# Bissmella/Small-object-detection-transformers

Measured on AMD Instinct MI355X. Metric: images/sec (1024x1024 RGB+IR) train fwd+bwd, higher is better.
Workload: dtype bf16; 1 GPU; SRyolo_MF.yaml (model.yaml graph), batch 8/GPU @ 1024x1024 RGB+IR, fwd + hand-written bwd + fused SGD-nesterov/weight-decay + EMA step, loss = YOLOv5 ComputeLoss (CIoU + BCE, device kernels), 32 synthetic boxes/image, random-init weights; global_batch=8, parallelism=dp1

## Files before the change

### include/sodt_hip.h

```cpp
#ifndef SODT_HIP_H
#define SODT_HIP_H
#include <stddef.h>
#include <stdint.h>

#ifdef __cplusplus
extern "C" {
#endif

typedef struct ihipStream_t* sodt_stream_t;

#define SODT_F32 0
#define SODT_BF16 1
#define SODT_MAX_SEG 9

typedef struct {
  const void* p;
  int ld;
  int klen;
  int dy, dx;
  int mul, shr;
  int Hi, Wi;
} sodt_seg;

typedef struct {
// ... 18 lines not shown
#define SODT_EPI_DRELU 4096

typedef struct {
  sodt_aspec a;
  const void* W; int ldw;
  void* C; int ldc;
  void* C2; int ldc2;
  const float* bias;
  const void* R; int ldr; int rmod;
  const void* aux; int ldaux;
  double* stats;
  const float* scale; const float* shift;
  int M, N, K, flags;
  int oscatter, omul, ody, odx, OH, OW;
  int det_na, det_no, det_hw;
} sodt_gemm_args;

int sodt_gemm_nt(const sodt_gemm_args* g, int dtype, sodt_stream_t st);
int sodt_gemm_set_variant(int force_tiled);

typedef struct {
  const void* dY; int ldy;
  sodt_aspec x;
  float* dW; int lddw;
  float* dbias;
  int M, N, K;
  int kperm_c, kperm_t;
  int splits;
  float* partial;
  long partial_floats;
} sodt_gemm_tn_args;

int sodt_gemm_tn(const sodt_gemm_tn_args* g, int dtype, sodt_stream_t st);

int sodt_layernorm_fwd(const void* x, const float* gamma, const float* beta, void* y, float* stats,
                       int M, int C, int dtype, sodt_stream_t st);
int sodt_layernorm_bwd(const void* dy, const void* x, const float* stats, const float* gamma,
                       const void* dres, void* dx, float* dgamma, float* dbeta,
                       int M, int C, int dtype, sodt_stream_t st);

int sodt_window_attn_fwd(const void* qkv, const float* bias_t, void* out, float* lse,
                         int B, int H, int W, int C, int heads, int ws, int shift,
                         int dtype, sodt_stream_t st);
int sodt_window_attn_bwd(const void* qkv, const float* bias_t, const void* out, const void* dout,
                         const float* lse, void* dqkv, float* dbias_t, float* dq_acc,
                         int B, int H, int W, int C, int heads, int ws, int shift,
                         int dtype, sodt_stream_t st);

int sodt_bilinear_up2_fwd(const void* x, void* y, int ldy, int B, int H, int W, int C, int dtype, sodt_stream_t st);
int sodt_bilinear_up2_bwd(const void* dy, int lddy, void* dx, const void* relu_out, int B, int H, int W, int C, int dtype,
                          sodt_stream_t st);
int sodt_pixel_shuffle2(const void* in, void* out, int B, int H, int W, int C, int inverse, int dtype, sodt_stream_t st);
int sodt_add_rows(void* dst, int ldd, int dcol, const void* src, int lds, int scol, long M, int C, int dtype, sodt_stream_t st);
int sodt_nchw_f32_from_rows(const void* rows, int ld, float* y, int B, int C, int H, int W, int dtype, sodt_stream_t st);
int sodt_rows_from_nchw_f32(const float* y, void* rows, int ld, int B, int C, int H, int W, int dtype, sodt_stream_t st);

int sodt_conv3x3_c64n8_fwd(const void* x, const void* w, const float* bias, void* y, float* y_nchw, int B, int H, int W, int cout, int dtype,
                           sodt_stream_t st);
int sodt_conv3x3_c64n8_dgrad(const void* dy, const float* dy_nchw, const void* wT, void* dx, int B, int H, int W, int cout, int dtype,
                             sodt_stream_t st);
int sodt_conv3x3_c64n8_wgrad(const void* dy, const float* dy_nchw, const void* x, float* dw, float* db, float* scratch, int B, int H, int W,
                             int cout, int dtype, sodt_stream_t st);
long sodt_conv3x3_c64n8_wgrad_scratch_bytes(void);

typedef struct {
  int w_row_stride, w_row_off;
// ... 195 lines not shown
```

### small-object-detection-transformers_amd/_lib.py

```python
from __future__ import annotations

import ctypes as C
import os

HERE = os.path.dirname(os.path.abspath(__file__))
DEFAULT_LIB_PATH = os.path.join(HERE, "libsodt_hip.so")
LIB_PATH = os.environ.get("SODT_LIB_PATH") or DEFAULT_LIB_PATH
DIAGNOSTIC_ENV = ("SODT_LIB_PATH", "SODT_HG_DBG", "SODT_WMSA_ONE_WAVE")


def overrides():
    return {k: os.environ[k] for k in DIAGNOSTIC_ENV if os.environ.get(k)}

MAX_SEG = 9
F32, BF16 = 0, 1
U8 = 2
SR_MODES = {"IR": 0, "RGB": 1, "RGB+IR": 2}
EPI_BIAS, EPI_RESID, EPI_GELU_DUAL, EPI_DGELU = 1, 2, 4, 8
EPI_STATS, EPI_AFFINE_SILU, EPI_DETECT, EPI_OUT_F32 = 16, 32, 64, 128
EPI_GELU, EPI_DGELU_RC, EPI_RELU, EPI_DRELU = 256, 512, 2048, 4096
STATS_REPL = 16


class Seg(C.Structure):
    _fields_ = [("p", C.c_void_p), ("ld", C.c_int), ("klen", C.c_int), ("dy", C.c_int), ("dx", C.c_int),
                ("mul", C.c_int), ("shr", C.c_int), ("Hi", C.c_int), ("Wi", C.c_int)]


class ASpec(C.Structure):
    _fields_ = [("s", Seg * MAX_SEG), ("nseg", C.c_int), ("spatial", C.c_int), ("Ho", C.c_int), ("Wo", C.c_int)]


class GemmArgs(C.Structure):
    _fields_ = [("a", ASpec),
                ("W", C.c_void_p), ("ldw", C.c_int),
                ("C", C.c_void_p), ("ldc", C.c_int),
                ("C2", C.c_void_p), ("ldc2", C.c_int),
                ("bias", C.c_void_p),
                ("R", C.c_void_p), ("ldr", C.c_int), ("rmod", C.c_int),
                ("aux", C.c_void_p), ("ldaux", C.c_int),
                ("stats", C.c_void_p),
                ("scale", C.c_void_p), ("shift", C.c_void_p),
                ("M", C.c_int), ("N", C.c_int), ("K", C.c_int), ("flags", C.c_int),
                ("oscatter", C.c_int), ("omul", C.c_int), ("ody", C.c_int), ("odx", C.c_int),
                ("OH", C.c_int), ("OW", C.c_int),
                ("det_na", C.c_int), ("det_no", C.c_int), ("det_hw", C.c_int)]


class GemmTnArgs(C.Structure):
    _fields_ = [("dY", C.c_void_p), ("ldy", C.c_int),
                ("x", ASpec),
                ("dW", C.c_void_p), ("lddw", C.c_int),
                ("dbias", C.c_void_p),
                ("M", C.c_int), ("N", C.c_int), ("K", C.c_int),
                ("kperm_c", C.c_int), ("kperm_t", C.c_int), ("splits", C.c_int),
                ("partial", C.c_void_p), ("partial_floats", C.c_long)]


class StepCtl(C.Structure):
    _fields_ = [("acc_sumsq", C.c_double), ("acc_found", C.c_uint), ("ticket", C.c_uint),
                ("sumsq", C.c_double), ("grad_norm", C.c_double), ("step", C.c_longlong),
                ("found_inf", C.c_float), ("inv_scale_eff", C.c_float), ("clip_coef", C.c_float), ("skip", C.c_int),
                ("reserved", C.c_int * 2)]


class PrepDesc(C.Structure):
    _fields_ = [("src", C.c_void_p), ("dst", C.c_void_p),
                ("d0", C.c_int), ("d1", C.c_int), ("d2", C.c_int),
                ("p0", C.c_int), ("p1", C.c_int), ("p2", C.c_int),
                ("dst_ld", C.c_int), ("inner_ld", C.c_int)]


_P, _I, _L, _F = C.c_void_p, C.c_int, C.c_long, C.c_float
class Conv3Geo(C.Structure):
    _fields_ = [("w_row_stride", C.c_int), ("w_row_off", C.c_int), ("in_mul", C.c_int), ("in_i", C.c_int), ("in_j", C.c_int),
                ("out_mul", C.c_int), ("out_i", C.c_int), ("out_j", C.c_int)]


SIGNATURES = {
    "sodt_nms_candidates": [_P, _I, _I, C.c_float, _I, _P, _P, _I, _P, _P],
    "sodt_nms_workspace_bytes": [_L, C.POINTER(C.c_size_t)],
    "sodt_nms_select": [_P, _I, _P, _L, C.c_float, _I, _P, C.c_size_t, _P, _P, _P, _P],
    "sodt_wbf_candidates": [_P, _I, _I, _I, _F, _F, _P, _P, _P, _P, _P, _P],
    "sodt_wbf_fuse_workspace_bytes": [_I, _L, C.POINTER(C.c_size_t)],
    "sodt_wbf_fuse": [_P, _P, _P, _P, _P, _P, _I, _L, C.POINTER(C.c_double), _I, C.c_double, _F, _I, _I, _I, _P, C.c_size_t,
                      _P, _P, _P, _P, _P, _P],
    "sodt_eval_match_workspace_bytes": [_I, _L, _L, C.POINTER(C.c_size_t)],
    "sodt_eval_match": [_P, _P, _I, _L, _P, _L, _P, C.POINTER(C.c_float), _P, C.c_size_t, _P, _P, _P],
    "sodt_ap_per_class_workspace_bytes": [_L, _L, _I, C.POINTER(C.c_size_t)],
    "sodt_ap_per_class": [_P, _P, _P, _L, _P, _L, _I, _P, C.c_size_t, _P, _P, _P, _P, _P, _P, _P, _P],
    "sodt_confusion_update_workspace_bytes": [_I, _L, _L, C.POINTER(C.c_size_t)],
    "sodt_confusion_update": [_P, _P, _I, _L, _P, _L, _P, _I, _F, _F, _P, C.c_size_t, _P, _P, _P],
    "sodt_gemm_nt": [C.POINTER(GemmArgs), _I, _P],
    "sodt_gemm_tn": [C.POINTER(GemmTnArgs), _I, _P],
    "sodt_layernorm_fwd": [_P, _P, _P, _P, _P, _I, _I, _I, _P],
    "sodt_layernorm_bwd": [_P, _P, _P, _P, _P, _P, _P, _P, _I, _I, _I, _P],
    "sodt_window_attn_fwd": [_P, _P, _P, _P, _I, _I, _I, _I, _I, _I, _I, _I, _P],
    "sodt_window_attn_bwd": [_P, _P, _P, _P, _P, _P, _P, _P, _I, _I, _I, _I, _I, _I, _I, _I, _P],
    "sodt_wmsa_pack": [_P, _P, _P, _P, _P, _P, _P, _P, _P, _P, _I, _I, _I, _I, _P],
    "sodt_wmsa_block_fwd": [_P, _P, _P, _P, _P, _P, _P, _P, _P, _P, _I, _I, _I, _I, _I, _I, _I, _I, _P],
    "sodt_window_attn_bwd_wm": [_P, _P, _P, _P, _P, _P, _I, _I, _I, _I, _I, _I, _I, _I, _P],
    "sodt_wmsa_block_bwd": [_P, _P, _P, _P, _P, _P, _P, _I, _I, _I, _I, _I, _I, _I, _I, _P],
    "sodt_frontend_fwd": [_P, _P, _L, _P, _P, _P, _P, _P, _I, _I, _I, _I, _P],
    "sodt_frontend_bwd": [_P, _P, _L, _P, _P, _P, _P, _P, _P, _P, _P, _P, _I, _I, _I, _P, _L, _I, _P],
    "sodt_patch_embed4_fwd": [_P, _P, _L, _P, _P, _P, _I, _I, _P],
    "sodt_patch_embed4_bwd": [_P, _P, _L, _P, _P, _P, _I, _I, _P],
    "sodt_cross_attn_ln_fwd": [_P, _P, _P, _P, _I, _I, _I, _I, _I, _P],
    "sodt_cross_attn_ln_bwd": [_P, _P, _P, _P, _P, _P, _I, _I, _I, _I, _I, _P],
    "sodt_bn_finalize": [_P, _P, _P, _P, _L, _I, _F, _F, _P],
    "sodt_bn_affine": [_P, _P, _P, _P, _P, _I, _P],
    "sodt_bn_silu_fwd": [_P, _P, _P, _P, _P, _I, _L, _I, _I, _P],
    "sodt_bn_silu_bwd_reduce": [_P, _I, _P, _P, _P, _P, _P, _L, _I, _I, _P],
    "sodt_bn_silu_bwd_apply": [_P, _I, _P, _P, _P, _P, _P, _P, _P, _P, _L, _I, _I, _P],
    "sodt_copy_rows": [_P, _I, _P, _I, _I, _I, _I, _I, _I, _I, _P],
    "sodt_gather_sum_rows": [_P, _I, _P, _I, _I, _I, _I, _I, _I, _I, _I, _P],
    "sodt_detect_unpermute": [_P, _P, _I, _I, _I, _I, _I, _I, _P],
    "sodt_detect_decode": [_P, _P, _P, _I, _I, _I, _I, _I, _F, _P],
    "sodt_prep_weights": [_P, _I, _I, _I, _P],
    "sodt_transpose_f32": [_P, _P, _I, _I, _I, _P],
    "sodt_cast": [_P, _P, _L, _I, _I, _P],
    "sodt_batch_sum": [_P, _P, _I, _L, _I, _P],
    "sodt_memset_zero": [_P, _L, _P],
    "sodt_gemm_set_variant": [_I],
    "sodt_maxpool5_fwd": [_P, _I, _P, _I, _P, _I, _I, _I, _I, _I, _P],
    "sodt_maxpool5_bwd": [_P, _I, _P, _P, _I, _I, _I, _I, _I, _I, _I, _P],
    "sodt_yolo_loss_workspace_bytes": [_L, _I, _I, C.POINTER(C.c_size_t)],
    "sodt_yolo_loss": [_P, _P, _I, _P, _I, _I, _I, _I, _I, _F, _F, _F, _F, _F, _F, _F, _P, C.c_size_t, _P, _P, _P],
# ... 75 lines not shown
```

### small-object-detection-transformers_amd/engine.py

```python
from __future__ import annotations

import os

import ctypes as C
from typing import Dict, List, Optional, Tuple

import warnings

import torch

from . import _lib as L
from . import ops
from .ops import SegSpec

HEADS = 12
E = "image_encoder."
TAPS2 = ((0, 0), (0, 1), (1, 0), (1, 1))
TAPS3 = tuple((dy, dx) for dy in (-1, 0, 1) for dx in (-1, 0, 1))
MERGE = ((0, 0), (1, 0), (0, 1), (1, 1))
USE_HIPGRAPH = os.environ.get("SODT_HIPGRAPH", "0") == "1"


class Plan:
    def __init__(self, B, S, dt, training, dev):
# ... 99 lines not shown
        return None, None, None, None, None


class Engine:
    def __init__(self, model):
        self.model = model
        self.params: Dict[str, torch.nn.Parameter] = dict(model.named_parameters())
        self.buffers: Dict[str, torch.Tensor] = dict(model.named_buffers())
        p0 = next(iter(self.params.values()))
        if not p0.is_cuda:
            raise RuntimeError("move the model to the GPU first: the engine has no CPU path")
        for n, p in self.params.items():
            if p.dtype != torch.float32:
                raise RuntimeError(f"master parameters must be float32 (got {p.dtype} for {n}); call model.float()")
        self.dev = p0.device
        enc = model.image_encoder
        self.img_t = enc.pos_embed.shape[1]
        det = model.detect[-1]
        self.na, self.no, self.nc = det.na, det.no, det.nc
        self.det_np = (det.na * det.no + 15) // 16 * 16
        self.fused = not any(type(m).__name__ == "BatchNorm2d" for m in model.detect.modules())
        self.sr = bool(getattr(model, "sr", False))
        self._check_head()
        self.plans: Dict[Tuple, Plan] = {}
        self.probes_fwd: Optional[dict] = None
        self.probes_bwd: Optional[dict] = None
        self.prep: Dict[torch.dtype, dict] = {}
        self._build_grad_buffer()
        self._build_param_buffer()
        self._anchor = torch.zeros(1, device=self.dev, requires_grad=True)
        self.ddp = None
        self.use_fused_wmsa = True
        self.use_fused_mlp = True
        self.convmlp_fold_maxc = 384
        self.use_direct_conv3 = True
        self._tn_scratch = torch.empty(16 << 20, dtype=torch.float32, device=self.dev)
        ops.set_tn_scratch(self._tn_scratch)

    def _check_head(self):
        from . import model as M
        d = self.model.detect
        enc_c = (256, 256, 512)
        vals = {j: ([(("enc", j), enc_c[j], 0)], j) for j in range(3)}
        units, rules = [], {}
        uses: Dict[tuple, int] = {}

        def resolve(f, yi):
            j = yi - 1 if f == -1 else f
            if not isinstance(j, int) or j not in vals or j >= yi:
                raise NotImplementedError(f"head row {yi - 3}: input {f!r} does not name an earlier feature-list entry")
            return j
        if not isinstance(d[-1], M.Detect) or d[-1].nl != 1:
            raise NotImplementedError("the head must end in a one-layer Detect (models/model.yaml:74)")
        for k, m in enumerate(d):
            yi, kind = 3 + k, type(m).__name__
            if kind in ("Conv", "C3", "SPP"):
                if not isinstance(m.f, int):
                    raise NotImplementedError(f"head row {k}: {kind} takes one input")
                parts, level = vals[resolve(m.f, yi)]
                c1 = sum(c for _, c, _ in parts)
                if kind == "Conv":
                    kk, c2 = m.conv.kernel_size[0], m.conv.out_channels
                    if m.conv.in_channels != c1:
                        raise NotImplementedError(f"head row {k}: Conv expects {m.conv.in_channels} channels, graph gives {c1}")
                    if kk == 3 and len(parts) * 9 > L.MAX_SEG:
                        raise NotImplementedError(f"head row {k}: a 3x3 Conv on a concatenation needs {len(parts) * 9} K-segments (max {L.MAX_SEG})")
# ... 493 lines not shown
        elif pre in P["cmlp"]:
            cm = P["cmlp"][pre]
            ops.convmlp_compose(p[pre + "mlp.fc1.weight"], p[pre + "mlp.fc1.bias"], p[pre + "mlp.conv1.weight"], p[pre + "mlp.conv1.bias"],
                                cm["weff"], cm["weffT"], cm["beff"], cm["vtap"], Cc)
            cp = plan.buf(tag + ".cp", (M, Cc))
            ca = plan.buf(tag + ".ca", (M, Cc))
            segs = [SegSpec(xn2, Cc, 0, dy, dx, 1, 0, H, W) for (dy, dx) in TAPS2]
            ops.gemm_nt(segs, cm["weff"], cp, M, Cc, 4 * Cc, spatial=(H, W), bias=cm["beff"], gelu_out=ca)
            ops.convmlp_border_fix(cp, ca, cm["vtap"], B, H, W, Cc)
            ops.gemm_nt([SegSpec(ca)], w[pre + "mlp.fc2.weight"], xo, M, Cc, Cc, bias=p[pre + "mlp.fc2.bias"], resid=xm)
        else:
            u = plan.buf(tag + ".u", (M, Cc))
            ops.gemm_nt([SegSpec(xn2)], w[pre + "mlp.fc1.weight"], u, M, Cc, Cc, bias=p[pre + "mlp.fc1.bias"])
            cp = plan.buf(tag + ".cp", (M, Cc))
            ca = plan.buf(tag + ".ca", (M, Cc))
            segs = [SegSpec(u, Cc, 0, dy, dx, 1, 0, H, W) for (dy, dx) in TAPS2]
            ops.gemm_nt(segs, w[pre + "mlp.conv1.weight"], cp, M, Cc, 4 * Cc, spatial=(H, W), bias=p[pre + "mlp.conv1.bias"],
                        gelu_out=ca)
            ops.gemm_nt([SegSpec(ca)], w[pre + "mlp.fc2.weight"], xo, M, Cc, Cc, bias=p[pre + "mlp.fc2.bias"], resid=xm)
        plan.saved[tag] = dict(x_in=x_in, geo=(B, H, W, Cc, ws, shift), fused=fused, wpk=wpk, pad=(Hp, Wp) if padded else None)
        return xo

    def _block_bwd(self, plan, P, tag, blk, dY, dX):
        ops.set_tag(tag + ".bwd")
        p, wT, g, b = self.params, P["wT"], self.g, plan.bufs
        pre = E + tag + "."
        sv = plan.saved[tag]
        B, H, W, Cc, ws, shift = sv["geo"]
        M = B * H * W
        x_in = sv["x_in"]
        xm, xn2, xn1, ao = b[tag + ".xm"], b[tag + ".xn2"], b[tag + ".xn1"], b[tag + ".ao"]
        dxn = plan.buf(f"g.dxn.{Cc}", (M, Cc))
        dxm = plan.buf(f"g.dxm.{Cc}", (M, Cc))
        if blk.mlp.linear:
            ha = b[tag + ".ha"]
            dh = plan.buf(f"g.dh.{Cc}", (M, 4 * Cc))
            ops.gemm_tn(dY, [SegSpec(ha)], g[pre + "mlp.fc2.weight"], M, Cc, 4 * Cc, dbias=g[pre + "mlp.fc2.bias"])
            if (tag + ".hp") in b:
                ops.gemm_nt([SegSpec(dY)], wT[pre + "mlp.fc2.weight"], dh, M, 4 * Cc, Cc, dgelu_aux=b[tag + ".hp"])
            else:
                ops.gemm_nt([SegSpec(xn2), SegSpec(dY)], P["wcat"][pre + "mlp.fc1.weight"], dh, M, 4 * Cc, 2 * Cc,
                            bias=p[pre + "mlp.fc1.bias"], dgelu_rc=True)
            ops.gemm_tn(dh, [SegSpec(xn2)], g[pre + "mlp.fc1.weight"], M, 4 * Cc, Cc, dbias=g[pre + "mlp.fc1.bias"])
            dln2 = (dh, 4 * Cc)
        elif pre in P["cmlp"]:
            cm = P["cmlp"][pre]
            cp, ca = b[tag + ".cp"], b[tag + ".ca"]
            dc = plan.buf(f"g.dc.{Cc}", (M, Cc))
            ops.gemm_tn(dY, [SegSpec(ca)], g[pre + "mlp.fc2.weight"], M, Cc, Cc, dbias=g[pre + "mlp.fc2.bias"])
            ops.gemm_nt([SegSpec(dY)], wT[pre + "mlp.fc2.weight"], dc, M, Cc, Cc, dgelu_aux=cp)
            scr = plan.buf(f"g.cmlp.{Cc}", (Cc * 4 * Cc + 4 * Cc,), torch.float32)
            dweff, colsum, bs = scr[: Cc * 4 * Cc].view(Cc, 4 * Cc), scr[Cc * 4 * Cc: Cc * 4 * Cc + Cc], scr[Cc * 4 * Cc + Cc:].view(3, Cc)
            ops.zero_(scr)
            segs = [SegSpec(xn2, Cc, 0, dy, dx, 1, 0, H, W) for (dy, dx) in TAPS2]
            ops.gemm_tn(dc, segs, dweff, M, Cc, 4 * Cc, spatial=(H, W), dbias=colsum)
            ops.convmlp_border_sums(dc, bs, B, H, W, Cc)
            ops.convmlp_decompose(dweff, colsum, bs, p[pre + "mlp.fc1.weight"], p[pre + "mlp.fc1.bias"], p[pre + "mlp.conv1.weight"],
                                  g[pre + "mlp.conv1.weight"], g[pre + "mlp.conv1.bias"], g[pre + "mlp.fc1.weight"], g[pre + "mlp.fc1.bias"], Cc)
            dln2 = None
        else:
            u, cp, ca = b[tag + ".u"], b[tag + ".cp"], b[tag + ".ca"]
            dc = plan.buf(f"g.dc.{Cc}", (M, Cc))
            du = plan.buf(f"g.du.{Cc}", (M, Cc))
            ops.gemm_tn(dY, [SegSpec(ca)], g[pre + "mlp.fc2.weight"], M, Cc, Cc, dbias=g[pre + "mlp.fc2.bias"])
            ops.gemm_nt([SegSpec(dY)], wT[pre + "mlp.fc2.weight"], dc, M, Cc, Cc, dgelu_aux=cp)
            segs = [SegSpec(u, Cc, 0, dy, dx, 1, 0, H, W) for (dy, dx) in TAPS2]
            ops.gemm_tn(dc, segs, g[pre + "mlp.conv1.weight"], M, Cc, 4 * Cc, spatial=(H, W), dbias=g[pre + "mlp.conv1.bias"],
                        kperm=(Cc, 4))
            segs = [SegSpec(dc, Cc, 0, -dy, -dx, 1, 0, H, W) for (dy, dx) in TAPS2]
            ops.gemm_nt(segs, wT[pre + "mlp.conv1.weight"], du, M, Cc, 4 * Cc, spatial=(H, W))
            ops.gemm_tn(du, [SegSpec(xn2)], g[pre + "mlp.fc1.weight"], M, Cc, Cc, dbias=g[pre + "mlp.fc1.bias"])
            dln2 = (du, Cc)
        if dln2 is None:
            segs = [SegSpec(dc, Cc, 0, -dy, -dx, 1, 0, H, W) for (dy, dx) in TAPS2]
            ops.gemm_nt(segs, cm["weffT"], dxn, M, Cc, 4 * Cc, spatial=(H, W))
            ops.layernorm_bwd(dxn, xm, b[tag + ".st2"], p[pre + "norm2.weight"], dY, dxm, g[pre + "norm2.weight"], g[pre + "norm2.bias"], M, Cc)
        else:
            ops.gemm_nt([SegSpec(dln2[0])], wT[pre + "mlp.fc1.weight"], dxn, M, Cc, dln2[1])
            ops.layernorm_bwd(dxn, xm, b[tag + ".st2"], p[pre + "norm2.weight"], dY, dxm, g[pre + "norm2.weight"], g[pre + "norm2.bias"], M, Cc)
        if sv.get("pad"):
            self._padded_attn_bwd(plan, P, tag, pre, sv, dxm, dxn, dX)
            return
        ops.gemm_tn(dxm, [SegSpec(ao)], g[pre + "attn.proj.weight"], M, Cc, Cc, dbias=g[pre + "attn.proj.bias"])
        dao = dxn
        ops.gemm_nt([SegSpec(dxm)], wT[pre + "attn.proj.weight"], dao, M, Cc, Cc)
        dqkv = plan.buf(f"g.dqkv.{Cc}", (M, 3 * Cc))
        L2 = 2 * ws - 1
        dbt = plan.buf(f"g.dbt.{L2}", (HEADS, L2 * L2), torch.float32, zero=True)
        if sv["fused"] and plan.dt == torch.bfloat16:
            ops.wmsa_block_bwd(xn1, sv["wpk"], P["bias_t"][pre + "attn.relative_position_bias_table"], dao, b[tag + ".lsew"],
                               dqkv, dbt, B, H, W, Cc, HEADS, ws, shift)
        elif sv["fused"]:
            ops.window_attn_bwd_wm(b[tag + ".qkvw"], P["bias_t"][pre + "attn.relative_position_bias_table"], dao, b[tag + ".lsew"],
                                   dqkv, dbt, B, H, W, Cc, HEADS, ws, shift)
        else:
            scratch = plan.buf(f"g.attn_scratch.{Cc}", (M * (Cc + HEADS),), torch.float32, zero=True) if ws * ws > 64 else None
            ops.window_attn_bwd(b[tag + ".qkv"], P["bias_t"][pre + "attn.relative_position_bias_table"], ao, dao, b[tag + ".lse"], dqkv,
                                dbt, scratch, B, H, W, Cc, HEADS, ws, shift)
        ops.transpose_f32(dbt, g[pre + "attn.relative_position_bias_table"], HEADS, L2 * L2, accumulate=2)
        ops.gemm_tn(dqkv, [SegSpec(xn1)], g[pre + "attn.qkv.weight"], M, 3 * Cc, Cc, dbias=g[pre + "attn.qkv.bias"])
        ops.gemm_nt([SegSpec(dqkv)], wT[pre + "attn.qkv.weight"], dxn, M, Cc, 3 * Cc)
        ops.layernorm_bwd(dxn, x_in, b[tag + ".st1"], p[pre + "norm1.weight"], dxm, dX, g[pre + "norm1.weight"], g[pre + "norm1.bias"], M, Cc)

    def _padded_attn_bwd(self, plan, P, tag, pre, sv, dxm, dxn, dX):
        p, wT, g, b = self.params, P["wT"], self.g, plan.bufs
        B, H, W, Cc, ws, _ = sv["geo"]
        Hp, Wp = sv["pad"]
        M, Mp = B * H * W, B * Hp * Wp
        aop, qkv, lse = b[tag + ".aop"], b[tag + ".qkv"], b[tag + ".lse"]
        ops.gemm_tn(dxm, [SegSpec(aop, Cc, 0, 0, 0, 1, 0, Hp, Wp)], g[pre + "attn.proj.weight"], M, Cc, Cc, spatial=(H, W),
                    dbias=g[pre + "attn.proj.bias"])
        daop = plan.buf(f"g.daop.{Cc}", (Mp, Cc))
        ops.gemm_nt([SegSpec(dxm, Cc, 0, 0, 0, 1, 0, H, W)], wT[pre + "attn.proj.weight"], daop, Mp, Cc, Cc, spatial=(Hp, Wp))
        dqkv = plan.buf(f"g.dqkvp.{Cc}", (Mp, 3 * Cc))
        L2 = 2 * ws - 1
        dbt = plan.buf(f"g.dbt.{L2}", (HEADS, L2 * L2), torch.float32, zero=True)
        scratch = plan.buf(f"g.attn_scratchp.{Cc}", (Mp * (Cc + HEADS),), torch.float32, zero=True) if ws * ws > 64 else None
        ops.window_attn_bwd(qkv, P["bias_t"][pre + "attn.relative_position_bias_table"], aop, daop, lse, dqkv, dbt, scratch,
# ... 371 lines not shown
```

### small-object-detection-transformers_amd/ops.py

```python
from __future__ import annotations

import ctypes as C
from typing import List, Optional, Sequence, Tuple

import torch

from . import _lib as L

_lib = L.load()

_active_recorder: Optional[list] = None


class Recorder:

    def __init__(self):
        self.calls: List[Tuple] = []
        self.keep: List = []

    def __enter__(self):
        global _active_recorder
        assert _active_recorder is None, "nested recorders are not supported"
        _active_recorder = self.calls
        return self
# ... 199 lines not shown
    return max(1, min(M // 256 if M >= 256 else 1, max(1, slots // tiles)))


_tn_scratch: Optional[torch.Tensor] = None


def set_tn_scratch(t: Optional[torch.Tensor]) -> None:
    global _tn_scratch
    assert t is None or (t.dtype == torch.float32 and t.is_contiguous())
    _tn_scratch = t


def gemm_tn(dY: torch.Tensor, segs: Sequence[SegSpec], dW: torch.Tensor, M: int, N: int, K: int, *,
            ldy: Optional[int] = None, y_off: int = 0, spatial: Optional[Tuple[int, int]] = None,
            dbias: Optional[torch.Tensor] = None, lddw: Optional[int] = None, kperm: Optional[Tuple[int, int]] = None,
            splits: Optional[int] = None) -> None:
    g = L.GemmTnArgs()
    g.dY = dY.data_ptr() + y_off * dY.element_size()
    g.ldy = dY.shape[-1] if ldy is None else ldy
    _fill_aspec(g.x, segs, spatial)
    assert dW.dtype == torch.float32
    g.dW = dW.data_ptr()
    g.lddw = K if lddw is None else lddw
    g.dbias = _p(dbias)
    g.M, g.N, g.K = M, N, K
    if kperm is not None:
        g.kperm_c, g.kperm_t = kperm
    g.splits = tn_splits(M, N, K, dY.dtype == torch.bfloat16) if splits is None else splits
    if _tn_scratch is not None and _tn_scratch.device == dY.device and g.splits > 1:
        g.partial, g.partial_floats = _tn_scratch.data_ptr(), _tn_scratch.numel()
    _launch("sodt_gemm_tn", C.byref(g), dt_code(dY))


def layernorm_fwd(x, gamma, beta, y, stats, M, Cc):
    _launch("sodt_layernorm_fwd", _p(x), _p(gamma), _p(beta), _p(y), _p(stats), M, Cc, dt_code(x))


def layernorm_bwd(dy, x, stats, gamma, dres, dx, dgamma, dbeta, M, Cc):
    _launch("sodt_layernorm_bwd", _p(dy), _p(x), _p(stats), _p(gamma), _p(dres), _p(dx), _p(dgamma), _p(dbeta),
            M, Cc, dt_code(x))


def window_attn_fwd(qkv, bias_t, out, lse, B, H, W, Cc, heads, ws, shift):
    _launch("sodt_window_attn_fwd", _p(qkv), _p(bias_t), _p(out), _p(lse), B, H, W, Cc, heads, ws, shift, dt_code(qkv))


def window_attn_bwd(qkv, bias_t, out, dout, lse, dqkv, dbias_t, scratch, B, H, W, Cc, heads, ws, shift):
    _launch("sodt_window_attn_bwd", _p(qkv), _p(bias_t), _p(out), _p(dout), _p(lse), _p(dqkv), _p(dbias_t), _p(scratch),
            B, H, W, Cc, heads, ws, shift, dt_code(qkv))


def wmsa_pack_bytes(Cc: int, heads: int, ws: int, dtype_code: int) -> int:
    return int(_lib.sodt_wmsa_pack_bytes(Cc, heads, ws, dtype_code))


def wmsa_pack(qkv_w, qkv_b, proj_w, proj_b, table, n1w, n1b, n2w, n2b, wpk, Cc, heads, ws):
    _launch("sodt_wmsa_pack", _p(qkv_w), _p(qkv_b), _p(proj_w), _p(proj_b), _p(table), _p(n1w), _p(n1b), _p(n2w), _p(n2b),
            _p(wpk), Cc, heads, ws, L.BF16 if wpk.dtype == torch.bfloat16 else L.F32)


def wmsa_block_fwd(x, wpk, xm, xn2, st1, st2, xn1, qkvw, lsew, ao, B, H, W, Cc, heads, ws, shift):
    _launch("sodt_wmsa_block_fwd", _p(x), _p(wpk), _p(xm), _p(xn2), _p(st1), _p(st2), _p(xn1), _p(qkvw), _p(lsew), _p(ao),
            B, H, W, Cc, heads, ws, shift, dt_code(x))


def window_attn_bwd_wm(qkvw, bias_t, dout, lsew, dqkv, dbias_t, B, H, W, Cc, heads, ws, shift):
# ... 402 lines not shown
```

Measured before the change: 213.8 images/sec.

## Fuse square 192x192 linear backward dX and dW GEMMs into one kernel

Adds a HIP kernel that computes both the input gradient (dY·W, with an optional dGELU epilogue) and the weight/bias gradient (Xᵀ·dY) for 192x192 linears in a single pass. dY and X tiles are streamed through LDS once with a 3-stage global_load_lds pipeline, and the weight stays resident in LDS. Per-split partial sums are then combined by a separate reduce kernel. It replaces separate gemm_tn and gemm_nt launches for attn.proj and the conv-MLP fc2 backward at C=192, aiming to cut dY re-reads and launch count, and falls back to the old path when the shape or alignment checks fail.

```diff
diff --git a/include/sodt_hip.h b/include/sodt_hip.h
--- a/include/sodt_hip.h
+++ b/include/sodt_hip.h
@@ -74,6 +74,22 @@
 } sodt_gemm_tn_args;
 
 int sodt_gemm_tn(const sodt_gemm_tn_args* g, int dtype, sodt_stream_t st);
+
+typedef struct {
+  const void* dY; int ldy;
+  const void* X; int ldx;
+  const void* wT; int ldw;
+  const void* aux; int ldaux;
+  void* dX; int lddx;
+  float* dW; int lddw;
+  float* dbias;
+  int M, N, K, flags;
+  int splits;
+  float* partial;
+  long partial_floats;
+} sodt_linbwd_args;
+
+int sodt_linear_bwd_sq(const sodt_linbwd_args* g, int dtype, sodt_stream_t st);
 
 int sodt_layernorm_fwd(const void* x, const float* gamma, const float* beta, void* y, float* stats,
                        int M, int C, int dtype, sodt_stream_t st);
diff --git a/small-object-detection-transformers_amd/_lib.py b/small-object-detection-transformers_amd/_lib.py
--- a/small-object-detection-transformers_amd/_lib.py
+++ b/small-object-detection-transformers_amd/_lib.py
@@ -54,6 +54,19 @@
                 ("dbias", C.c_void_p),
                 ("M", C.c_int), ("N", C.c_int), ("K", C.c_int),
                 ("kperm_c", C.c_int), ("kperm_t", C.c_int), ("splits", C.c_int),
+                ("partial", C.c_void_p), ("partial_floats", C.c_long)]
+
+
+class LinBwdArgs(C.Structure):
+    _fields_ = [("dY", C.c_void_p), ("ldy", C.c_int),
+                ("X", C.c_void_p), ("ldx", C.c_int),
+                ("wT", C.c_void_p), ("ldw", C.c_int),
+                ("aux", C.c_void_p), ("ldaux", C.c_int),
+                ("dX", C.c_void_p), ("lddx", C.c_int),
+                ("dW", C.c_void_p), ("lddw", C.c_int),
+                ("dbias", C.c_void_p),
+                ("M", C.c_int), ("N", C.c_int), ("K", C.c_int), ("flags", C.c_int),
+                ("splits", C.c_int),
                 ("partial", C.c_void_p), ("partial_floats", C.c_long)]
 
 
@@ -93,6 +106,7 @@
     "sodt_confusion_update": [_P, _P, _I, _L, _P, _L, _P, _I, _F, _F, _P, C.c_size_t, _P, _P, _P],
     "sodt_gemm_nt": [C.POINTER(GemmArgs), _I, _P],
     "sodt_gemm_tn": [C.POINTER(GemmTnArgs), _I, _P],
+    "sodt_linear_bwd_sq": [C.POINTER(LinBwdArgs), _I, _P],
     "sodt_layernorm_fwd": [_P, _P, _P, _P, _P, _I, _I, _I, _P],
     "sodt_layernorm_bwd": [_P, _P, _P, _P, _P, _P, _P, _P, _I, _I, _I, _P],
     "sodt_window_attn_fwd": [_P, _P, _P, _P, _I, _I, _I, _I, _I, _I, _I, _I, _P],
diff --git a/small-object-detection-transformers_amd/csrc/linbwd.hip b/small-object-detection-transformers_amd/csrc/linbwd.hip
--- /dev/null
+++ b/small-object-detection-transformers_amd/csrc/linbwd.hip
@@ -0,0 +1,364 @@
+#include "gemm_epi.h"
+
+namespace {
+
+typedef __attribute__((address_space(3))) void lds_void;
+typedef __attribute__((address_space(1))) const void glb_void;
+typedef __attribute__((ext_vector_type(4))) unsigned int u32x4;
+
+constexpr int LB_C = 192;
+constexpr int LB_ROWB = LB_C * 2;
+constexpr int LB_WBYTES = LB_C * LB_ROWB;
+constexpr int LB_ROWS = 32, LB_NST = 3;
+constexpr int LB_IMG = LB_ROWS * LB_ROWB;
+constexpr int LB_STAGE = 2 * LB_IMG;
+constexpr int LB_LDS = LB_WBYTES + LB_NST * LB_STAGE;
+
+__device__ uint4 lb_zero16[4];
+
+__device__ __forceinline__ uint32_t lb_lds_addr(const void* p) { return (uint32_t)(uintptr_t)(lds_void*)p; }
+
+template <int OFF> __device__ __forceinline__ u32x4 lb_rd128(uint32_t addr) {
+  u32x4 v;
+  asm volatile("ds_read_b128 %0, %1 offset:%2" : "=v"(v) : "v"(addr), "n"(OFF));
+  return v;
+}
+template <int OFF> __device__ __forceinline__ uint2 lb_rd_tr(uint32_t addr) {
+  typedef __attribute__((ext_vector_type(2))) unsigned int u32x2;
+  u32x2 t;
+  asm volatile("ds_read_b64_tr_b16 %0, %1 offset:%2" : "=v"(t) : "v"(addr), "n"(OFF));
+  uint2 v; v.x = t.x; v.y = t.y;
+  return v;
+}
+__device__ __forceinline__ u32x4 lb_frag_tr(uint32_t addr) {
+  const uint2 lo = lb_rd_tr<0>(addr), hi = lb_rd_tr<4 * LB_ROWB>(addr);
+  u32x4 r; r.x = lo.x; r.y = lo.y; r.z = hi.x; r.w = hi.y;
+  return r;
+}
+#define LB_LGKM0() do { asm volatile("s_waitcnt lgkmcnt(0)" ::: "memory"); __builtin_amdgcn_sched_barrier(0); } while (0)
+
+__device__ __forceinline__ void lb_mma(f32x4& acc, const u32x4& a, const u32x4& b) {
+  union { u32x4 u; bf16x8 v; } ua, ub;
+  ua.u = a; ub.u = b;
+  acc = __builtin_amdgcn_mfma_f32_16x16x32_bf16(ua.v, ub.v, acc, 0, 0, 0);
+}
+
+template <bool DG>
+__global__ __launch_bounds__(512) void linbwd_sq_kernel(const sodt_linbwd_args g, float* __restrict__ partial, float* __restrict__ bpartial) {
+  extern __shared__ __attribute__((aligned(16))) unsigned char dsm[];
+  const int tid = threadIdx.x, lane = tid & 63, wid = __builtin_amdgcn_readfirstlane(tid >> 6);
+  const int wr = wid >> 1, wc = wid & 1;
+  const int fr = lane & 15, fg = lane >> 4;
+  const uint32_t lbase = lb_lds_addr(dsm);
+
+  const int split = xcd_remap(blockIdx.x, gridDim.x);
+  const long rows_per = (((g.M + g.splits - 1) / g.splits) + LB_ROWS - 1) / LB_ROWS * LB_ROWS;
+  const long mbeg = (long)split * rows_per;
+  const long mend = (mbeg + rows_per < g.M) ? (mbeg + rows_per) : g.M;
+  if (mbeg >= mend) return;
+  const int nrows = (int)(mend - mbeg);
+  const int nsteps = (nrows + LB_ROWS - 1) / LB_ROWS;
+
+  {
+    uint4 wv[9];
+#pragma unroll
+    for (int e = 0; e < 9; ++e) {
+      const int id = tid + 512 * e, r = id / 24, c = id - r * 24;
+      wv[e] = *(const uint4*)((const bf16*)g.wT + (long)r * g.ldw + 8 * c);
+    }
+#pragma unroll
+    for (int e = 0; e < 9; ++e) {
+      const int id = tid + 512 * e, r = id / 24, c = id - r * 24;
+      const int f = ((r >> 1) & 1) | (((r >> 3) & 3) << 1);
+      *(uint4*)(dsm + r * LB_ROWB + ((c ^ f) << 4)) = wv[e];
+    }
+  }
+  __syncthreads();
+
+  const unsigned char* zero = (const unsigned char*)lb_zero16;
+  const bool ximg = wid >= 4;
+  const int jb = 3 * (wid & 3);
+  const long ld_src = ximg ? g.ldx : g.ldy;
+  const unsigned char* src0 = (const unsigned char*)(ximg ? g.X : g.dY);
+  auto chunk_row = [&](int e) { return (64 * (jb + e) + lane) / 24; };
+  auto chunk_col = [&](int e) {
+    const int id = 64 * (jb + e) + lane;
+    const int r2 = id / 24, c2 = id - r2 * 24;
+    const int sw2 = ((r2 >> 1) & 1) | (((r2 >> 3) & 1) << 1);
+    return ((((c2 >> 1) ^ sw2) << 1) | (c2 & 1)) << 3;
+  };
+  const int drow0 = chunk_row(0), drow1 = chunk_row(1), drow2 = chunk_row(2);
+  const unsigned char* cur0 = src0 + (((mbeg + drow0) * ld_src + chunk_col(0)) << 1);
+  const unsigned char* cur1 = src0 + (((mbeg + drow1) * ld_src + chunk_col(1)) << 1);
+  const unsigned char* cur2 = src0 + (((mbeg + drow2) * ld_src + chunk_col(2)) << 1);
+  const long dstep = (long)LB_ROWS * ld_src * 2;
+  const uint32_t ddst = LB_WBYTES + (ximg ? LB_IMG : 0) + jb * 1024;
+  int rel = 0;
+  auto issue = [&](int slot) {
+    const uint32_t dst = ddst + slot * LB_STAGE;
+    const unsigned char* s0 = rel + drow0 < nrows ? cur0 : zero;
+    const unsigned char* s1 = rel + drow1 < nrows ? cur1 : zero;
+    const unsigned char* s2 = rel + drow2 < nrows ? cur2 : zero;
+    __builtin_amdgcn_global_load_lds((glb_void*)s0, (lds_void*)(dsm + dst), 16, 0, 0);
+    __builtin_amdgcn_global_load_lds((glb_void*)s1, (lds_void*)(dsm + dst + 1024), 16, 0, 0);
+    __builtin_amdgcn_global_load_lds((glb_void*)s2, (lds_void*)(dsm + dst + 2048), 16, 0, 0);
+    rel += LB_ROWS;
+    cur0 += dstep; cur1 += dstep; cur2 += dstep;
+  };
+
+  const int q_ = fr >> 2, p_ = fr & 3;
+  const int frow = 8 * fg + q_;
+  const int swQ = (q_ >> 1) | ((fg & 1) << 1);
+  const uint32_t tbase = lbase + LB_WBYTES + frow * LB_ROWB + 8 * p_;
+  uint32_t pa[3], qa[6];
+#pragma unroll
+  for (int i = 0; i < 3; ++i) pa[i] = tbase + (((wr * 3 + i) ^ swQ) << 5);
+#pragma unroll
+  for (int j = 0; j < 6; ++j) qa[j] = tbase + LB_IMG + (((wc * 6 + j) ^ swQ) << 5);
+
+  const int s2 = ((fr >> 1) & 1) | (((fr >> 3) & 1) << 1);
+  const uint32_t yRd0 = lbase + LB_WBYTES + fr * LB_ROWB + (((fg >> 1) ^ s2) << 5) + ((fg & 1) << 4);
+  const uint32_t yRd1 = lbase + LB_WBYTES + fr * LB_ROWB + (((2 + (fg >> 1)) ^ s2) << 5) + ((fg & 1) << 4);
+  const int fW = ((fr >> 1) & 1) | (((fr >> 2) & 3) << 1);
+  const int wrow = 32 * (wid < 6 ? wid : 0) + 8 * (fr >> 2) + (fr & 3);
+  const uint32_t wRd0 = lbase + wrow * LB_ROWB + ((fg ^ fW) << 4);
+  const uint32_t wRd1 = lbase + wrow * LB_ROWB + (((4 + fg) ^ fW) << 4);
+  const bool nt_wave = wid < 6;
+  const int ocol = 32 * wid + 8 * fg;
+
+  const bool do_bias = g.dbias != nullptr && wc == 0;
+  u32x4 ones; ones.x = ones.y = ones.z = ones.w = 0x3F803F80u;
+
+  f32x4 acc[3][6], bacc[3];
+#pragma unroll
+  for (int i = 0; i < 3; ++i) {
+#pragma unroll
+    for (int j = 0; j < 6; ++j) acc[i][j] = f32x4{0.f, 0.f, 0.f, 0.f};
+    bacc[i] = f32x4{0.f, 0.f, 0.f, 0.f};
+  }
+
+  u32x4 pre0, pre1;
+  pre0.x = pre0.y = pre0.z = pre0.w = 0u; pre1 = pre0;
+  auto aux_ptr = [&](int stage, int u) {
+    long m = mbeg + (long)stage * LB_ROWS + 16 * u + fr;
+    if (m >= g.M) m = g.M - 1;
+    return (const bf16*)g.aux + m * g.ldaux + ocol;
+  };
+
+  issue(0);
+  if (DG && nt_wave) {
+    const bf16* a0 = aux_ptr(0, 0);
+    const bf16* a1 = aux_ptr(0, 1);
+    asm volatile("global_load_dwordx4 %0, %1, off" : "=v"(pre0) : "v"(a0) : "memory");
+    asm volatile("global_load_dwordx4 %0, %1, off" : "=v"(pre1) : "v"(a1) : "memory");
+  }
+  issue(1);
+  int slot = 0;
+  for (int s = 0; s < nsteps; ++s) {
+    if (DG && nt_wave) asm volatile("s_waitcnt vmcnt(5)" ::: "memory");
+    else asm volatile("s_waitcnt vmcnt(3)" ::: "memory");
+    __builtin_amdgcn_s_barrier();
+    asm volatile("" ::: "memory");
+    const uint32_t so = slot * LB_STAGE;
+
+    if (nt_wave) {
+      f32x4 na00 = f32x4{0.f, 0.f, 0.f, 0.f}, na01 = na00, na10 = na00, na11 = na00;
+#define LB_NT_RD(KS, YB, WB, T)                                                                       \
+      const u32x4 fy0##T = lb_rd128<128 * ((KS) >> 1)>(YB + so);                                      \
+      const u32x4 fy1##T = lb_rd128<128 * ((KS) >> 1) + 16 * LB_ROWB>(YB + so);                       \
+      const u32x4 fw0##T = lb_rd128<128 * ((KS) >> 1)>(WB);                                           \
+      const u32x4 fw1##T = lb_rd128<128 * ((KS) >> 1) + 4 * LB_ROWB>(WB);
+#define LB_NT_MM(T)                                                                                   \
+      lb_mma(na00, fw0##T, fy0##T); lb_mma(na01, fw1##T, fy0##T);                                     \
+      lb_mma(na10, fw0##T, fy1##T); lb_mma(na11, fw1##T, fy1##T);
+      {
+        LB_NT_RD(0, yRd0, wRd0, a) LB_NT_RD(1, yRd1, wRd1, b)
+        LB_LGKM0();
+        LB_NT_MM(a) LB_NT_MM(b)
+      }
+      {
+        LB_NT_RD(2, yRd0, wRd0, a) LB_NT_RD(3, yRd1, wRd1, b)
+        LB_LGKM0();
+        LB_NT_MM(a) LB_NT_MM(b)
+      }
+      {
+        LB_NT_RD(4, yRd0, wRd0, a) LB_NT_RD(5, yRd1, wRd1, b)
+        LB_LGKM0();
+        LB_NT_MM(a) LB_NT_MM(b)
+      }
+#undef LB_NT_RD
+#undef LB_NT_MM
+      if (DG) {
+        asm volatile("s_waitcnt vmcnt(3)" : "+v"(pre0), "+v"(pre1) :: "memory");
+        __builtin_amdgcn_sched_barrier(0);
+      }
+      const int r0 = s * LB_ROWS + fr;
+      {
+        float v[8];
+#pragma unroll
+        for (int r = 0; r < 4; ++r) { v[r] = na00[r]; v[4 + r] = na01[r]; }
+        if (DG) {
+          float x[8];
+          uint4 pu; pu.x = pre0.x; pu.y = pre0.y; pu.z = pre0.z; pu.w = pre0.w;
+          unpack<bf16>(pu, x);
+#pragma unroll
+          for (int j = 0; j < 8; ++j) v[j] *= dgelu_t<bf16>(x[j]);
+        }
+        if (r0 < nrows) *(uint4*)((bf16*)g.dX + (mbeg + r0) * g.lddx + ocol) = pack<bf16>(v);
+      }
+      {
+        float v[8];
+#pragma unroll
+        for (int r = 0; r < 4; ++r) { v[r] = na10[r]; v[4 + r] = na11[r]; }
+        if (DG) {
+          float x[8];
+          uint4 pu; pu.x = pre1.x; pu.y = pre1.y; pu.z = pre1.z; pu.w = pre1.w;
+          unpack<bf16>(pu, x);
+#pragma unroll
+          for (int j = 0; j < 8; ++j) v[j] *= dgelu_t<bf16>(x[j]);
+        }
+        if (r0 + 16 < nrows) *(uint4*)((bf16*)g.dX + (mbeg + r0 + 16) * g.lddx + ocol) = pack<bf16>(v);
+      }
+      if (DG) {
+        __builtin_amdgcn_sched_barrier(0);
+        const bf16* a0 = aux_ptr(s + 1, 0);
+        const bf16* a1 = aux_ptr(s + 1, 1);
+        asm volatile("global_load_dwordx4 %0, %1, off" : "=v"(pre0) : "v"(a0) : "memory");
+        asm volatile("global_load_dwordx4 %0, %1, off" : "=v"(pre1) : "v"(a1) : "memory");
+      }
+    }
+    issue(slot == 0 ? LB_NST - 1 : slot - 1);
+
+    {
+      u32x4 fp[3], fq[6];
+#pragma unroll
+      for (int i = 0; i < 3; ++i) fp[i] = lb_frag_tr(pa[i] + so);
+#pragma unroll
+      for (int j = 0; j < 6; ++j) fq[j] = lb_frag_tr(qa[j] + so);
+      LB_LGKM0();
+#pragma unroll
+      for (int i = 0; i < 3; ++i)
+#pragma unroll
+        for (int j = 0; j < 6; ++j) lb_mma(acc[i][j], fp[i], fq[j]);
+      if (do_bias) {
+#pragma unroll
+        for (int i = 0; i < 3; ++i) lb_mma(bacc[i], fp[i], ones);
+      }
+    }
+    slot = slot == LB_NST - 1 ? 0 : slot + 1;
+  }
+  if (DG) asm volatile("s_waitcnt vmcnt(0)" : "+v"(pre0), "+v"(pre1) :: "memory");
+  else asm volatile("s_waitcnt vmcnt(0)" ::: "memory");
+  __builtin_amdgcn_sched_barrier(0);
+
+  if (partial) {
+    float* part = partial + (long)split * LB_C * LB_C + (wr * 48 + 4 * fg) * LB_C + wc * 96 + fr;
+#pragma unroll
+    for (int i = 0; i < 3; ++i)
+#pragma unroll
+      for (int j = 0; j < 6; ++j)
+#pragma unroll
+        for (int r = 0; r < 4; ++r) part[(16 * i + r) * LB_C + 16 * j] = acc[i][j][r];
+  } else {
+    float* d = g.dW + (long)(wr * 48 + 4 * fg) * g.lddw + wc * 96 + fr;
+#pragma unroll
+    for (int i = 0; i < 3; ++i)
+#pragma unroll
+      for (int j = 0; j < 6; ++j)
+#pragma unroll
+        for (int r = 0; r < 4; ++r) atomicAdd(d + (long)(16 * i + r) * g.lddw + 16 * j, acc[i][j][r]);
+  }
+  if (do_bias && fr == 0) {
+#pragma unroll
+    for (int i = 0; i < 3; ++i)
+#pragma unroll
+      for (int r = 0; r < 4; ++r) {
+        const int n = wr * 48 + 16 * i + 4 * fg + r;
+        if (bpartial) bpartial[(long)split * LB_C + n] = bacc[i][r];
+        else atomicAdd(g.dbias + n, bacc[i][r]);
+      }
+  }
+}
+
+__global__ __launch_bounds__(256) void linbwd_reduce_kernel(const float* __restrict__ partial, float* __restrict__ dW, int lddw, int live,
+                                                           const float* __restrict__ bpartial, float* __restrict__ dbias, int wblocks) {
+  __shared__ float4 red[4][64];
+  const bool bias = (int)blockIdx.x >= wblocks;
+  const float* src = bias ? bpartial : partial;
+  const long slice = bias ? LB_C : (long)LB_C * LB_C;
+  const long n4 = slice / 4;
+  const int c = threadIdx.x & 63, sg = threadIdx.x >> 6;
+  const long i = (long)(bias ? (int)blockIdx.x - wblocks : (int)blockIdx.x) * 64 + c;
+  float4 a = make_float4(0.f, 0.f, 0.f, 0.f);
+  if (i < n4) {
+    const float* p = src + i * 4;
+    int s = sg;
+    for (; s + 12 < live; s += 16) {
+      const float4 v0 = *(const float4*)(p + (long)s * slice), v1 = *(const float4*)(p + (long)(s + 4) * slice);
+      const float4 v2 = *(const float4*)(p + (long)(s + 8) * slice), v3 = *(const float4*)(p + (long)(s + 12) * slice);
+      a.x += (v0.x + v1.x) + (v2.x + v3.x); a.y += (v0.y + v1.y) + (v2.y + v3.y);
+      a.z += (v0.z + v1.z) + (v2.z + v3.z); a.w += (v0.w + v1.w) + (v2.w + v3.w);
+    }
+    for (; s < live; s += 4) {
+      const float4 v = *(const float4*)(p + (long)s * slice);
+      a.x += v.x; a.y += v.y; a.z += v.z; a.w += v.w;
+    }
+  }
+  red[sg][c] = a;
+  __syncthreads();
+  if (sg == 0 && i < n4) {
+    const float4 b1 = red[1][c], b2 = red[2][c], b3 = red[3][c];
+    a.x += b1.x + b2.x + b3.x; a.y += b1.y + b2.y + b3.y; a.z += b1.z + b2.z + b3.z; a.w += b1.w + b2.w + b3.w;
+    float* d;
+    if (bias) d = dbias + i * 4;
+    else { const int n = (int)((i * 4) / LB_C); d = dW + (long)n * lddw + (int)(i * 4 - (long)n * LB_C); }
+    float4 o = *(float4*)d;
+    o.x += a.x; o.y += a.y; o.z += a.z; o.w += a.w;
+    *(float4*)d = o;
+  }
+}
+
+template <bool DG>
+int launch_linbwd(const sodt_linbwd_args* g, float* partial, float* bpartial, hipStream_t st) {
+  static bool attr_set = false;
+  if (!attr_set) {
+    if (hipFuncSetAttribute((const void*)linbwd_sq_kernel<DG>, hipFuncAttributeMaxDynamicSharedMemorySize, LB_LDS) != hipSuccess) {
+      (void)hipGetLastError();
+      return SODT_EINVAL;
+    }
+    attr_set = true;
+  }
+  hipLaunchKernelGGL((linbwd_sq_kernel<DG>), dim3((unsigned)g->splits), dim3(512), LB_LDS, st, *g, partial, bpartial);
+  return hipGetLastError() == hipSuccess ? SODT_OK : SODT_EINVAL;
+}
+
+}
+
+extern "C" int sodt_linear_bwd_sq(const sodt_linbwd_args* g, int dtype, sodt_stream_t st) {
+  if (!g || dtype != SODT_BF16 || g->N != LB_C || g->K != LB_C || g->M <= 0 || g->splits < 1 || g->splits > 65535) return SODT_EINVAL;
+  if (!g->dY || !g->X || !g->wT || !g->dX || !g->dW) return SODT_EINVAL;
+  if (g->flags != 0 && g->flags != SODT_EPI_DGELU) return SODT_EINVAL;
+  if ((g->ldy % 8) || (g->ldx % 8) || (g->ldw % 8) || (g->lddx % 8) || (g->lddw % 4)) return SODT_EINVAL;
+  if (g->ldy < LB_C || g->ldx < LB_C || g->ldw < LB_C || g->lddx < LB_C || g->lddw < LB_C) return SODT_EINVAL;
+  if ((((uintptr_t)g->dY) | ((uintptr_t)g->X) | ((uintptr_t)g->wT) | ((uintptr_t)g->dX) | ((uintptr_t)g->dW)) & 15) return SODT_EINVAL;
+  if (g->dbias && (((uintptr_t)g->dbias) & 15)) return SODT_EINVAL;
+  if (g->flags & SODT_EPI_DGELU) {
+    if (!g->aux || (g->ldaux % 8) || g->ldaux < LB_C || (((uintptr_t)g->aux) & 15)) return SODT_EINVAL;
+  }
+  const long tile_floats = (long)g->splits * LB_C * LB_C;
+  const bool use_partial = g->partial && g->splits > 1 && tile_floats <= g->partial_floats && (((uintptr_t)g->partial) & 15) == 0;
+  float* partial = use_partial ? g->partial : nullptr;
+  float* bpartial = (use_partial && g->dbias && tile_floats + (long)g->splits * LB_C <= g->partial_floats) ? g->partial + tile_floats : nullptr;
+  const int rc = (g->flags & SODT_EPI_DGELU) ? launch_linbwd<true>(g, partial, bpartial, (hipStream_t)st)
+                                             : launch_linbwd<false>(g, partial, bpartial, (hipStream_t)st);
+  if (rc != SODT_OK) return rc;
+  if (use_partial) {
+    const long rows_per = ((((long)g->M + g->splits - 1) / g->splits) + LB_ROWS - 1) / LB_ROWS * LB_ROWS;
+    const int live = (int)(((long)g->M + rows_per - 1) / rows_per);
+    const int wblocks = LB_C * LB_C / 4 / 64;
+    hipLaunchKernelGGL(linbwd_reduce_kernel, dim3(wblocks + (bpartial ? 1 : 0)), dim3(256), 0, (hipStream_t)st, (const float*)partial,
+                       g->dW, g->lddw, live, (const float*)bpartial, g->dbias, wblocks);
+    if (hipGetLastError() != hipSuccess) return SODT_EINVAL;
+  }
+  return SODT_OK;
+}
diff --git a/small-object-detection-transformers_amd/engine.py b/small-object-detection-transformers_amd/engine.py
--- a/small-object-detection-transformers_amd/engine.py
+++ b/small-object-detection-transformers_amd/engine.py
@@ -155,6 +155,7 @@
         self.ddp = None
         self.use_fused_wmsa = True
         self.use_fused_mlp = True
+        self.use_fused_linbwd = True
         self.convmlp_fold_maxc = 384
         self.use_direct_conv3 = True
         self._tn_scratch = torch.empty(16 << 20, dtype=torch.float32, device=self.dev)
@@ -714,6 +715,7 @@
         xm, xn2, xn1, ao = b[tag + ".xm"], b[tag + ".xn2"], b[tag + ".xn1"], b[tag + ".ao"]
         dxn = plan.buf(f"g.dxn.{Cc}", (M, Cc))
         dxm = plan.buf(f"g.dxm.{Cc}", (M, Cc))
+        linbwd = self.use_fused_linbwd and not sv.get("pad") and plan.dt == torch.bfloat16 and Cc == 192
         if blk.mlp.linear:
             ha = b[tag + ".ha"]
             dh = plan.buf(f"g.dh.{Cc}", (M, 4 * Cc))
@@ -729,8 +731,10 @@
             cm = P["cmlp"][pre]
             cp, ca = b[tag + ".cp"], b[tag + ".ca"]
             dc = plan.buf(f"g.dc.{Cc}", (M, Cc))
-            ops.gemm_tn(dY, [SegSpec(ca)], g[pre + "mlp.fc2.weight"], M, Cc, Cc, dbias=g[pre + "mlp.fc2.bias"])
-            ops.gemm_nt([SegSpec(dY)], wT[pre + "mlp.fc2.weight"], dc, M, Cc, Cc, dgelu_aux=cp)
+            if not (linbwd and ops.linear_bwd_sq(dY, ca, wT[pre + "mlp.fc2.weight"], dc, g[pre + "mlp.fc2.weight"], M,
+                                                 dbias=g[pre + "mlp.fc2.bias"], dgelu_aux=cp)):
+                ops.gemm_tn(dY, [SegSpec(ca)], g[pre + "mlp.fc2.weight"], M, Cc, Cc, dbias=g[pre + "mlp.fc2.bias"])
+                ops.gemm_nt([SegSpec(dY)], wT[pre + "mlp.fc2.weight"], dc, M, Cc, Cc, dgelu_aux=cp)
             scr = plan.buf(f"g.cmlp.{Cc}", (Cc * 4 * Cc + 4 * Cc,), torch.float32)
             dweff, colsum, bs = scr[: Cc * 4 * Cc].view(Cc, 4 * Cc), scr[Cc * 4 * Cc: Cc * 4 * Cc + Cc], scr[Cc * 4 * Cc + Cc:].view(3, Cc)
             ops.zero_(scr)
@@ -744,8 +748,10 @@
             u, cp, ca = b[tag + ".u"], b[tag + ".cp"], b[tag + ".ca"]
             dc = plan.buf(f"g.dc.{Cc}", (M, Cc))
             du = plan.buf(f"g.du.{Cc}", (M, Cc))
-            ops.gemm_tn(dY, [SegSpec(ca)], g[pre + "mlp.fc2.weight"], M, Cc, Cc, dbias=g[pre + "mlp.fc2.bias"])
-            ops.gemm_nt([SegSpec(dY)], wT[pre + "mlp.fc2.weight"], dc, M, Cc, Cc, dgelu_aux=cp)
+            if not (linbwd and ops.linear_bwd_sq(dY, ca, wT[pre + "mlp.fc2.weight"], dc, g[pre + "mlp.fc2.weight"], M,
+                                                 dbias=g[pre + "mlp.fc2.bias"], dgelu_aux=cp)):
+                ops.gemm_tn(dY, [SegSpec(ca)], g[pre + "mlp.fc2.weight"], M, Cc, Cc, dbias=g[pre + "mlp.fc2.bias"])
+                ops.gemm_nt([SegSpec(dY)], wT[pre + "mlp.fc2.weight"], dc, M, Cc, Cc, dgelu_aux=cp)
             segs = [SegSpec(u, Cc, 0, dy, dx, 1, 0, H, W) for (dy, dx) in TAPS2]
             ops.gemm_tn(dc, segs, g[pre + "mlp.conv1.weight"], M, Cc, 4 * Cc, spatial=(H, W), dbias=g[pre + "mlp.conv1.bias"],
                         kperm=(Cc, 4))
@@ -763,9 +769,11 @@
         if sv.get("pad"):
             self._padded_attn_bwd(plan, P, tag, pre, sv, dxm, dxn, dX)
             return
-        ops.gemm_tn(dxm, [SegSpec(ao)], g[pre + "attn.proj.weight"], M, Cc, Cc, dbias=g[pre + "attn.proj.bias"])
         dao = dxn
-        ops.gemm_nt([SegSpec(dxm)], wT[pre + "attn.proj.weight"], dao, M, Cc, Cc)
+        if not (linbwd and ops.linear_bwd_sq(dxm, ao, wT[pre + "attn.proj.weight"], dao, g[pre + "attn.proj.weight"], M,
+                                             dbias=g[pre + "attn.proj.bias"])):
+            ops.gemm_tn(dxm, [SegSpec(ao)], g[pre + "attn.proj.weight"], M, Cc, Cc, dbias=g[pre + "attn.proj.bias"])
+            ops.gemm_nt([SegSpec(dxm)], wT[pre + "attn.proj.weight"], dao, M, Cc, Cc)
         dqkv = plan.buf(f"g.dqkv.{Cc}", (M, 3 * Cc))
         L2 = 2 * ws - 1
         dbt = plan.buf(f"g.dbt.{L2}", (HEADS, L2 * L2), torch.float32, zero=True)
diff --git a/small-object-detection-transformers_amd/ops.py b/small-object-detection-transformers_amd/ops.py
--- a/small-object-detection-transformers_amd/ops.py
+++ b/small-object-detection-transformers_amd/ops.py
@@ -255,6 +255,46 @@
     _launch("sodt_gemm_tn", C.byref(g), dt_code(dY))
 
 
+def linear_bwd_sq(dY: torch.Tensor, X: torch.Tensor, wT: torch.Tensor, dX: torch.Tensor, dW: torch.Tensor, M: int, *,
+                  dbias: Optional[torch.Tensor] = None, dgelu_aux: Optional[torch.Tensor] = None,
+                  ldy: Optional[int] = None, y_off: int = 0, ldx: Optional[int] = None, lddx: Optional[int] = None,
+                  lddw: Optional[int] = None, splits: Optional[int] = None) -> bool:
+    ts = [dY, X, wT, dX] + ([dgelu_aux] if dgelu_aux is not None else [])
+    if any(t.dtype != torch.bfloat16 for t in ts) or dW.dtype != torch.float32 or (dbias is not None and dbias.dtype != torch.float32):
+        return False
+    if tuple(wT.shape) != (192, 192) or X.shape[-1] < 192 or dX.shape[-1] < 192:
+        return False
+    g = L.LinBwdArgs()
+    g.dY = dY.data_ptr() + y_off * dY.element_size()
+    g.ldy = dY.shape[-1] if ldy is None else ldy
+    g.X, g.ldx = X.data_ptr(), (X.shape[-1] if ldx is None else ldx)
+    g.wT, g.ldw = wT.data_ptr(), wT.stride(0)
+    g.dX, g.lddx = dX.data_ptr(), (dX.shape[-1] if lddx is None else lddx)
+    g.dW, g.lddw = dW.data_ptr(), (192 if lddw is None else lddw)
+    g.dbias = _p(dbias)
+    g.M, g.N, g.K = M, 192, 192
+    if dgelu_aux is not None:
+        g.flags = L.EPI_DGELU
+        g.aux, g.ldaux = dgelu_aux.data_ptr(), dgelu_aux.shape[-1]
+    g.splits = linear_bwd_sq_splits(M) if splits is None else splits
+    if _tn_scratch is not None and _tn_scratch.device == dY.device and g.splits > 1:
+        g.partial, g.partial_floats = _tn_scratch.data_ptr(), _tn_scratch.numel()
+    fn = _lib.sodt_linear_bwd_sq
+    args = (C.byref(g), L.BF16)
+    rc = fn(*args, C.c_void_p(torch.cuda.current_stream().cuda_stream))
+    if rc == 1:
+        return False
+    if rc != 0:
+        raise RuntimeError(f"sodt_linear_bwd_sq failed with status {rc}")
+    if _active_recorder is not None:
+        _active_recorder.append((fn, args, "sodt_linear_bwd_sq", _tag))
+    return True
+
+
+def linear_bwd_sq_splits(M: int) -> int:
+    return max(1, min(M // 512, 256))
+
+
 def layernorm_fwd(x, gamma, beta, y, stats, M, Cc):
     _launch("sodt_layernorm_fwd", _p(x), _p(gamma), _p(beta), _p(y), _p(stats), M, Cc, dt_code(x))
 
```

After: 216.6 images/sec, median of 6. +1.3%, better.
